# yekaizhou/duet

Measured on AMD Instinct MI355X. Metric: SV support-read marks clustered+phased /sec; bit-exact phased_sv.vcf vs ref, higher is better.
Workload: dtype u32/u64 integer + f64 threshold compares; 1 GPU; BASELINE configs[1]: synthetic 1 contig, 1001116 SV marks / 100000 candidates / 159991 tagged reads, resident in HBM; step = ef_classify + ef_finalize_own, two launches (phasing, E/F; ef_seed_sort 0: ; marks_per_gpu=1001116, candidates_per_gpu=100000, reads_per_gpu=159991, parallelism=contig-sharded x1, svlen_thres=50, suppread_thres=2, device_preheat_steps=2600

## Files before the change

duet_amd/csrc/duet_ef.hip:

```cpp

#include <hip/hip_runtime.h>
#include <hip/hip_ext.h>
#include <stdint.h>
#include <stdio.h>
#include <stdlib.h>
#include <string.h>
#include <string>
#include <vector>

#include "duet_ef.h"
#include "duet_internal.h"

#pragma clang fp contract(off)

namespace {

#ifdef DUET_STAMPS
#define STAMP(k, i) do { if (threadIdx.x == 0 && p.stamps) p.stamps[((size_t)(k) * 65536 + blockIdx.x) * 8 + (i)] = wall_clock64(); } while (0)
#else
#define STAMP(k, i) do { } while (0)
#endif

#include "duet_seeds.hip.h"

// ... 1414 lines not shown
        const bool live = c < n_cands;
        const uint8_t code = live ? p.out_pred[c] : 0;
        const uint32_t ps_in = live ? p.out_ps[c] : 0;
        if (tid == 0) {
            const uint32_t last = min(c0 + 255u, n_cands - 1);
            const uint32_t k0 = (DYN && p.cand_contig) ? (uint32_t)p.cand_contig[c0] : p.blk_ctg[tile];
            uint32_t k1 = k0;
            while (last >= p.ctg_off[k1 + 1]) ++k1;
            uint32_t any = 0;
            for (uint32_t k = k0; k <= k1; ++k) any |= (p.n_one[k] == 0);
            const uint32_t n0 = p.n_one[k0];
            s_meta[0] = k0;
            s_meta[1] = (k0 == k1 && n0 > 0 && n0 <= kOneLds) ? n0 : kEmpty;
            s_meta[2] = any;
            s_meta[3] = p.ctg_off[k0] + k0 + 1;
        }
        __syncthreads();
        STAMP(2, 1);
        const uint32_t k0 = s_meta[0], n_lds = s_meta[1], any_empty = s_meta[2];
        const bool lds_mode = n_lds != kEmpty;
        if (lds_mode) {
            const uint32_t *src = p.onebuf + s_meta[3];
            for (uint32_t i = tid; i < n_lds; i += 256u) s_one[i] = src[i];
            __syncthreads();
        }
        STAMP(2, 2);
        if (live) finalize_candidate(p, c, code, ps_in, k0, lds_mode, s_one, n_lds, any_empty);
        if (!DYN) break;
        __syncthreads();
    }
}

constexpr uint32_t kOwnMaxTiles = 2048;
constexpr uint32_t kOwnTab = 2048;
constexpr uint32_t kOwnKeys = 1024;

struct OwnArgs {
    TileRecs recs;
    const uint64_t *seed_ent, *read_tag;
    const uint32_t *cand_pos, *cand_off, *cand_svread, *cand_refread, *mark_read, *c2rec;
    uint32_t *out_ps, *status;
    uint8_t *out_pred;
    uint32_t c_lo, c_hi;
};

template <class F>
__device__ __forceinline__ void own_each_entry(TileRecs recs, const uint64_t *seed_ent, uint32_t c_lo, uint32_t c_hi, uint32_t first,
                                               uint32_t stride, F f)
{
    const uint32_t b_lo = c_lo / kCandPerBlock, b_hi = (c_hi - 1) / kCandPerBlock;
    for (uint32_t b = b_lo + first; b <= b_hi; b += stride) {
        const ulonglong4 rec = recs[b];
        const uint32_t cnt = (uint32_t)rec.x;
        for (uint32_t j = 0; j < cnt; ++j) {
            const uint64_t e = j == 0 ? rec.y : (j == 1 ? rec.z : (j == 2 ? rec.w : seed_ent[(size_t)b * kCandPerBlock + j]));
            const uint32_t c = (uint32_t)(e >> 32);
            if (c >= c_lo && c < c_hi) f((uint32_t)e);
        }
    }
}

__device__ __forceinline__ uint32_t own_nearest_walk(const OwnArgs &a, uint32_t pos)
{
    uint32_t best = 0;
    int64_t bd = -1;
    own_each_entry(a.recs, a.seed_ent, a.c_lo, a.c_hi, 0u, 1u, [&](uint32_t ps) {
// ... 64 lines not shown
                    ++n;
                    const uint32_t hap = tag_hap(u), pc = tag_pc(u);
                    n1 += hap == 1 ? 1u : 0u; s1 += hap == 1 ? pc : 0u;
                    n2 += hap == 2 ? 1u : 0u; s2 += hap == 2 ? pc : 0u;
                });
                done_ps = g;
                if (n > best) {
                    best = n; ps = g;
                    v.hap1 = n1; v.hap2 = n2; v.t1 = s1; v.t2 = s2;
                    v.hap0 = v.allhap - n1 - n2;
                }
            });
        }
        if (v.hap1 == 0 && v.hap2 == 0) ps = own_nearest_walk(a, c_pos);
        a.out_pred[c] = (uint8_t)decide(2, v, me - mb, a.cand_svread[c], a.cand_refread[c]);
        a.out_ps[c] = ps;
        return;
    }
    a.out_pred[c] = (uint8_t)(code & 3u);
    a.out_ps[c] = own_nearest_walk(a, c_pos);
}

__device__ __forceinline__ uint32_t wave_max_u32(uint32_t v)
{
    v = max(v, (uint32_t)__builtin_amdgcn_update_dpp(0, (int)v, 0xB1, 0xF, 0xF, false));
    v = max(v, (uint32_t)__builtin_amdgcn_update_dpp(0, (int)v, 0x4E, 0xF, 0xF, false));
    v = max(v, (uint32_t)__builtin_amdgcn_update_dpp(0, (int)v, 0x124, 0xF, 0xF, false));
    v = max(v, (uint32_t)__builtin_amdgcn_update_dpp(0, (int)v, 0x128, 0xF, 0xF, false));
    v = max(v, (uint32_t)__builtin_amdgcn_update_dpp(0, (int)v, 0x142, 0xA, 0xF, false));
    v = max(v, (uint32_t)__builtin_amdgcn_update_dpp(0, (int)v, 0x143, 0xC, 0xF, false));
    return (uint32_t)__builtin_amdgcn_readlane((int)v, 63);
}

__device__ __forceinline__ void own_sort_set(const uint32_t *s_tab, uint32_t *s_key, uint32_t *s_one, uint32_t *s_part, uint32_t u)
{
    const uint32_t tid = threadIdx.x, lane = tid & 63u, wave = tid >> 6;
    uint32_t mv[kOwnTab / 256u], cnt = 0;
#pragma unroll
    for (uint32_t j = 0; j < kOwnTab / 256u; ++j) {
        mv[j] = s_tab[tid + 256u * j];
        cnt += mv[j] != kEmpty ? 1u : 0u;
    }
    uint32_t x = cnt;
#pragma unroll
    for (int d = 1; d < 64; d <<= 1) {
        const uint32_t y = __shfl_up(x, d, 64);
        if ((int)lane >= d) x += y;
    }
    if (lane == 63) s_part[wave] = x;
    __syncthreads();
    uint32_t at = x - cnt;
#pragma unroll
    for (uint32_t w = 0; w < 4; ++w) at += w < wave ? s_part[w] : 0u;
#pragma unroll
    for (uint32_t j = 0; j < kOwnTab / 256u; ++j)
        if (mv[j] != kEmpty) s_key[at++] = mv[j];
    const uint32_t U = (u + 63u) & ~63u, nblk = U >> 6;
    if (tid < U - u) s_key[u + tid] = kEmpty;
    __syncthreads();
    for (uint32_t b = wave; b < nblk; b += 4u) s_key[b * 64u + lane] = wave_sort64(s_key[b * 64u + lane], lane);
    __syncthreads();
    for (uint32_t i = tid; i < U; i += 256u) {
        const uint32_t me = s_key[i];
        uint32_t rank = 0;
        for (uint32_t b = 0; b < nblk; b += 4u) {
            const uint32_t *b0 = s_key + b * 64u, *b1 = s_key + min(b + 1u, nblk - 1u) * 64u;
            const uint32_t *b2 = s_key + min(b + 2u, nblk - 1u) * 64u, *b3 = s_key + min(b + 3u, nblk - 1u) * 64u;
            uint32_t p0 = 0, p1 = 0, p2 = 0, p3 = 0;
#pragma unroll
            for (uint32_t st = 32; st > 0; st >>= 1) {
                p0 += b0[p0 + st - 1u] < me ? st : 0u;
                p1 += b1[p1 + st - 1u] < me ? st : 0u;
                p2 += b2[p2 + st - 1u] < me ? st : 0u;
                p3 += b3[p3 + st - 1u] < me ? st : 0u;
            }
            p0 += b0[p0] < me ? 1u : 0u;
            p1 += b1[p1] < me ? 1u : 0u;
            p2 += b2[p2] < me ? 1u : 0u;
            p3 += b3[p3] < me ? 1u : 0u;
            rank += p0 + (b + 1u < nblk ? p1 : 0u) + (b + 2u < nblk ? p2 : 0u) + (b + 3u < nblk ? p3 : 0u);
        }
        if (me != kEmpty) s_one[rank] = me;
    }
    __syncthreads();
}

__device__ __forceinline__ void own_vote_from_marks(const uint32_t *mark_read, const uint64_t *read_tag, uint32_t mb, uint32_t me_,
                                                 const uint32_t *s_tab, Vote *vo, uint32_t *pso)
{
    auto each = [&](auto f) {
        for (uint32_t m0 = mb; m0 < me_; m0 += 8) {
            uint32_t r[8];
            uint64_t t[8];
#pragma unroll
            for (int j = 0; j < 8; ++j) r[j] = mark_read[m0 + j < me_ ? m0 + j : mb];
// ... 26 lines not shown
        uint32_t n = 0, n1 = 0, n2 = 0;
        uint64_t s1 = 0, s2 = 0;
        each([&](uint64_t u) {
            if (u == kUntagged || tag_pc(u) > kPcMax || tag_ps(u) != g) return;
            ++n;
            const uint32_t hap = tag_hap(u), pc = tag_pc(u);
            n1 += hap == 1 ? 1u : 0u; s1 += hap == 1 ? pc : 0u;
            n2 += hap == 2 ? 1u : 0u; s2 += hap == 2 ? pc : 0u;
        });
        done_ps = g;
        if (n > best) {
            best = n; ps = g;
            v.hap1 = n1; v.hap2 = n2; v.t1 = s1; v.t2 = s2;
            v.hap0 = v.allhap - n1 - n2;
        }
    });
    *vo = v;
    *pso = ps;
}

__device__ __forceinline__ bool own_probe(uint32_t *s_tab, uint32_t key, uint32_t h)
{
    for (uint32_t probes = 0; probes < kOwnTab; ++probes) {
        const uint32_t old = atomicCAS(&s_tab[h], kEmpty, key);
        if (old == kEmpty) return true;
        if (old == key) return false;
        h = (h + 1u) & (kOwnTab - 1u);
    }
    return false;
}

constexpr uint32_t kOwnWin = 64;

__global__ __launch_bounds__(256) void ef_finalize_own(const Params p)
{
    __shared__ uint32_t s_tab[kOwnTab];
    __shared__ uint32_t s_key[kOwnKeys];
    __shared__ uint32_t s_one[kOwnKeys];
    __shared__ uint32_t s_win[kOwnWin];
    __shared__ uint32_t s_mm[4][2];
    __shared__ uint32_t s_red[4][3];
    __shared__ uint32_t s_part[4];
    __shared__ uint32_t s_nwin;
    __shared__ __align__(8) uint32_t s_c2[kC2Quota * kC2Words];
    const uint32_t tid = threadIdx.x, lane = tid & 63u, wave = tid >> 6;
    STAMP(2, 0);
    if (blockIdx.x == 0 && tid == 0) p.status[1] = 0;
    const uint32_t n_cands = p.C;
    const uint32_t nK = p.n_small;
    auto coff = [&](uint32_t kk) -> uint32_t { return p.ctg_small[kk]; };
    const uint32_t tile = blockIdx.x;
    const uint32_t c0 = tile * 256u, c = c0 + tid;
    const bool live = c < n_cands;
    const uint32_t cl = live ? c : n_cands - 1u;
    const uint32_t last = min(c0 + 255u, n_cands - 1);
    const uint32_t keys_cap = (p.dbg & DUET_DBG_EF_OWN_SMALLTAB) ? 8u : kOwnKeys;
    const uint32_t win_cap = (p.dbg & DUET_DBG_EF_OWN_SMALLTAB) ? 2u : kOwnWin;
    const TileRecs recs{reinterpret_cast<const ulonglong4 *>(p.blk_rec)};
    constexpr uint32_t kPre = 2;
    static_assert(kPre == 2, "the overflow loop selects between rec[0] and rec[1]");
    ulonglong4 rec[kPre], ext[kPre];
    auto load_recs = [&](uint32_t b_lo, uint32_t b_hi) {
#pragma unroll
        for (uint32_t i = 0; i < kPre; ++i) {
            const uint32_t b = min(b_lo + tid + 256u * i, b_hi);
            rec[i] = recs[b];
            ext[i] = recs.second(b);
        }
    };
    const uint32_t code_ld = p.out_pred[cl], ps_ld = p.out_ps[cl], pos_ld = p.cand_pos[cl];
    const uint32_t o0_ld = p.cand_off[cl], o1_ld = p.cand_off[cl + 1u];
    const uint32_t sv_ld = p.cand_svread[cl], rf_ld = p.cand_refread[cl];
    constexpr uint32_t kPairs = kC2Quota * kC2Words / 2;
    const uint2 *c2src = reinterpret_cast<const uint2 *>(p.c2rec + (size_t)tile * kC2Quota * kC2Words);
    const uint2 a0 = c2src[tid], a1 = c2src[tid + 256u < kPairs ? tid + 256u : tid];
    uint32_t lo = 0, hi = nK;
    while (hi - lo > 1) {
        const uint32_t mid = (lo + hi) >> 1;
        if (coff(mid) <= c0) lo = mid; else hi = mid;
    }
    uint32_t k_first = lo;
    while (k_first < nK && coff(k_first) == coff(k_first + 1)) ++k_first;
    {
        const uint32_t kf = k_first < nK ? k_first : 0u;
        load_recs(coff(kf) / kCandPerBlock, (coff(kf + 1) - 1) / kCandPerBlock);
    }
    asm volatile("" ::"v"(code_ld), "v"(ps_ld), "v"(pos_ld), "v"(o0_ld), "v"(o1_ld), "v"(sv_ld), "v"(rf_ld), "v"(a0.x), "v"(a0.y),
                 "v"(a1.x), "v"(a1.y));
    {
        uint2 *dst = reinterpret_cast<uint2 *>(s_c2);
        dst[tid] = a0;
        if (tid + 256u < kPairs) dst[tid + 256u] = a1;
    }
    const uint32_t code = live ? code_ld : 0u, ps_in = live ? ps_ld : 0u, c_pos = live ? pos_ld : 0u;
    const uint32_t c_o0 = live ? o0_ld : 0u, c_o1 = live ? o1_ld : 0u;
    const uint32_t c_svread = live ? sv_ld : 0u, c_refread = live ? rf_ld : 0u;
    for (uint32_t k = lo; k < nK && coff(k) <= last; ++k) {
        const uint32_t c_lo = coff(k), c_hi = coff(k + 1);
        if (c_lo == c_hi) continue;
        const uint32_t b_lo = c_lo / kCandPerBlock, b_hi = (c_hi - 1) / kCandPerBlock;
        if (k != k_first) load_recs(b_lo, b_hi);
#pragma unroll
        for (uint32_t i = 0; i < kOwnTab / 256u; ++i) s_tab[tid + 256u * i] = kEmpty;
        if (tid == 0) s_nwin = 0;
        const bool mine = live && c >= c_lo && c < c_hi;
        const bool asks = mine && code >= 4u && !(code & kDivZero);
        {
            const uint32_t mn = wave_max_u32(asks ? ~c_pos : 0u), mx = wave_max_u32(asks ? c_pos + 1u : 0u);
            if (lane == 0) { s_mm[wave][0] = mn; s_mm[wave][1] = mx; }
        }
        lds_barrier();
        STAMP(2, 1);
        asm volatile("" ::"v"(rec[0].x), "v"(rec[1].x), "v"(rec[0].y), "v"(rec[1].y), "v"(rec[0].z), "v"(rec[1].z), "v"(rec[0].w),
                     "v"(rec[1].w), "v"(ext[0].x), "v"(ext[1].x), "v"(ext[0].y), "v"(ext[1].y), "v"(ext[0].z), "v"(ext[1].z),
                     "v"(ext[0].w), "v"(ext[1].w));
        uint32_t pmin, pmax;
        {
            const uint32_t a0 = max(max(s_mm[0][0], s_mm[1][0]), max(s_mm[2][0], s_mm[3][0]));
            const uint32_t a1 = max(max(s_mm[0][1], s_mm[1][1]), max(s_mm[2][1], s_mm[3][1]));
            pmin = a1 ? ~a0 : 0u;
            pmax = a1 ? a1 - 1u : 0u;
        }
        uint32_t fresh = 0, leftp = 0, rinv = 0;
        static_assert(kOwnTab == 1u << 11, "the hash takes 11 bits");
        auto slot_of = [](uint32_t key) -> uint32_t { return (key * 2654435761u) >> (32u - 11u); };
        auto count_new = [&](bool nw, uint32_t key) {
            fresh += nw ? 1u : 0u;
            leftp = max(leftp, (nw && key <= pmin) ? key + 1u : 0u);
            rinv = max(rinv, (nw && key >= pmax) ? ~key : 0u);
            if (nw && key > pmin && key < pmax) {
                const uint32_t at = atomicAdd(&s_nwin, 1u);
                if (at < kOwnWin) s_win[at] = key;
            }
        };
        auto insert = [&](uint64_t e) {
            const uint32_t cc = (uint32_t)(e >> 32), key = (uint32_t)e;
            if (cc >= c_lo && cc < c_hi) count_new(own_probe(s_tab, key, slot_of(key)), key);
        };
        uint32_t coll = 0;
        auto group = [&](const uint64_t (&e)[4], uint32_t first, uint32_t n_in, uint32_t cnt, uint32_t bit0) {
            uint32_t key[4], old[4];
            bool ok[4];
#pragma unroll
            for (uint32_t j = 0; j < 4; ++j) {
                const uint32_t cc = (uint32_t)(e[j] >> 32);
                key[j] = (uint32_t)e[j];
                ok[j] = j < n_in && first + j < cnt && cc >= c_lo && cc < c_hi;
                old[j] = kEmpty;
            }
#pragma unroll
            for (uint32_t j = 0; j < 4; ++j)
                if (ok[j]) old[j] = atomicCAS(&s_tab[slot_of(key[j])], kEmpty, key[j]);
#pragma unroll
            for (uint32_t j = 0; j < 4; ++j) {
                coll |= (ok[j] && old[j] != kEmpty && old[j] != key[j]) ? 1u << (bit0 + j) : 0u;
                count_new(ok[j] && old[j] == kEmpty, key[j]);
            }
        };
#pragma unroll
        for (uint32_t i = 0; i < kPre; ++i) {
            const uint32_t cnt = b_lo + tid + 256u * i <= b_hi ? (uint32_t)rec[i].x : 0u;
            if (__any(cnt > 0u)) {
                const uint64_t e[4] = {rec[i].y, rec[i].z, rec[i].w, 0ull};
                group(e, 0u, 3u, cnt, 7u * i);
            }
            if (__any(cnt > 3u)) {
                const uint64_t e[4] = {ext[i].x, ext[i].y, ext[i].z, ext[i].w};
                group(e, 3u, 4u, cnt, 7u * i + 3u);
            }
        }
        while (coll) {
            const uint32_t j = (uint32_t)__ffs(coll) - 1u;
            coll &= coll - 1u;
            uint32_t key = 0;
#pragma unroll
            for (uint32_t i = 0; i < kPre; ++i) {
                key = j == 7u * i + 0u ? (uint32_t)rec[i].y : key;
                key = j == 7u * i + 1u ? (uint32_t)rec[i].z : key;
                key = j == 7u * i + 2u ? (uint32_t)rec[i].w : key;
                key = j == 7u * i + 3u ? (uint32_t)ext[i].x : key;
                key = j == 7u * i + 4u ? (uint32_t)ext[i].y : key;
                key = j == 7u * i + 5u ? (uint32_t)ext[i].z : key;
                key = j == 7u * i + 6u ? (uint32_t)ext[i].w : key;
            }
            count_new(own_probe(s_tab, key, (slot_of(key) + 1u) & (kOwnTab - 1u)), key);
        }
        auto overflow = [&](uint32_t b, uint32_t cnt, uint32_t from) {
            constexpr uint32_t kLong = 24;
            if (cnt > from && cnt <= kLong) {
                const uint64_t *ov = p.seed_ent + (size_t)b * kCandPerBlock;
#pragma unroll 1
                for (uint32_t j = from; j < cnt; j += 4) {
                    uint64_t e[4];
#pragma unroll
                    for (uint32_t t = 0; t < 4; ++t) e[t] = ov[min(j + t, cnt - 1u)];
#pragma unroll
                    for (uint32_t t = 0; t < 4; ++t)
                        if (j + t < cnt) insert(e[t]);
                }
            }
            unsigned long long todo = __ballot(cnt > kLong);
            while (todo) {
                const uint32_t h = (uint32_t)__ffsll((long long)todo) - 1u;
                todo &= todo - 1ull;
                const uint32_t b_h = (uint32_t)__builtin_amdgcn_readlane((int)b, h), cnt_h = (uint32_t)__builtin_amdgcn_readlane((int)cnt, h);
                const uint64_t *ov = p.seed_ent + (size_t)b_h * kCandPerBlock;
                for (uint32_t j = from + lane; j < cnt_h; j += 64u) insert(ov[j]);
            }
        };
#pragma unroll 1
        for (uint32_t i = 0, b0 = b_lo; b0 <= b_hi; ++i, b0 += 256u) {
            const uint32_t b = b0 + tid;
            uint32_t cnt, from = 7u;
            if (i < kPre) {
                cnt = b <= b_hi ? (uint32_t)(i == 0 ? rec[0].x : rec[1].x) : 0u;
            } else {
                ulonglong4 r = {0, 0, 0, 0};
                if (b <= b_hi) r = recs[b];
                cnt = (uint32_t)r.x;
                if (cnt > 0) insert(r.y);
                if (cnt > 1) insert(r.z);
                if (cnt > 2) insert(r.w);
                from = 3u;
            }
            overflow(b, cnt, from);
        }
        {
            const uint32_t l = wave_max_u32(leftp), r = wave_max_u32(rinv), o = wave_sum(fresh);
            if (lane == 0) { s_red[wave][0] = l; s_red[wave][1] = r; s_red[wave][2] = o; }
        }
        lds_barrier();
        STAMP(2, 2);
        const uint32_t u = s_red[0][2] + s_red[1][2] + s_red[2][2] + s_red[3][2];
        const uint32_t Lp = max(max(s_red[0][0], s_red[1][0]), max(s_red[2][0], s_red[3][0]));
        const uint32_t Ri = max(max(s_red[0][1], s_red[1][1]), max(s_red[2][1], s_red[3][1]));
        const uint32_t n_win = s_nwin;
        const bool over = u > keys_cap;
        const bool sorted = !over && n_win > win_cap;
        if (sorted) own_sort_set(s_tab, s_key, s_one, s_part, u);
        STAMP(2, 5);
        auto nearest = [&](uint32_t pos) -> uint32_t {
            if (sorted) return nearest_seed(s_one, u, pos);
            uint32_t best = 0;
            int64_t bd = -1;
            auto look = [&](uint32_t v) {
                const int64_t d = llabs((int64_t)pos - (int64_t)v);
                if (bd < 0 || d < bd || (d == bd && v > best)) { bd = d; best = v; }
            };
            if (Lp) look(Lp - 1u);
            if (Ri) look(~Ri);
            for (uint32_t i = 0; i < n_win; ++i) look(s_win[i]);
            return best;
        };
        auto member = [&](uint32_t key) -> bool {
            uint32_t h = (key * 2654435761u) >> (32u - 11u);
            for (;;) {
                const uint32_t v = s_tab[h];
                if (v == key) return true;
                if (v == kEmpty) return false;
                h = (h + 1u) & (kOwnTab - 1u);
            }
        };
        if (mine) {
            if (u == 0) {
                if (code != 0) p.out_pred[c] = 0;
                if (ps_in != 0) p.out_ps[c] = 0;
            } else if (code >= 4u) {
                if (code & kDivZero) {
                    atomicOr(&p.status[0], 1u);
                    p.out_pred[c] = 0;
                    p.out_ps[c] = 0;
                } else if (over) {
                    const OwnArgs a = {recs, p.seed_ent, p.read_tag, p.cand_pos, p.cand_off, p.cand_svread, p.cand_refread, p.mark_read, p.c2rec,
                                       p.out_ps, p.status, p.out_pred, c_lo, c_hi};
                    finalize_candidate_walk(a, c, code, ps_in);
                } else if (code & kClass2Slow) {
                    Vote v;
                    uint32_t ps;
                    own_vote_from_marks(p.mark_read, p.read_tag, c_o0, c_o1, s_tab, &v, &ps);
                    if (v.hap1 == 0 && v.hap2 == 0) ps = nearest(c_pos);
                    p.out_pred[c] = (uint8_t)decide(2, v, c_o1 - c_o0, c_svread, c_refread);
                    p.out_ps[c] = ps;
                } else if (code & kClass2) {
                    uint32_t w[kC2Words];
                    const uint32_t own0 = tile * kC2Quota;
                    if (ps_in >= own0 && ps_in < own0 + kC2Quota) {
#pragma unroll
                        for (int i = 0; i < kC2Words; ++i) w[i] = s_c2[(ps_in - own0) * kC2Words + i];
                    } else {
                        const uint32_t *rec2 = p.c2rec + (size_t)ps_in * kC2Words;
#pragma unroll
                        for (int i = 0; i < kC2Words; ++i) w[i] = rec2[i];
                    }
                    Vote v = {0, 0, 0, 0, 0, 0};
                    uint32_t ps = 0, best = 0;
                    v.allhap = w[0];
                    const uint32_t ng = w[1];
#pragma unroll
                    for (int g = 0; g < kC2Groups; ++g) {
                        if ((uint32_t)g < ng && w[2 + 6 * g + 1] > best && member(w[2 + 6 * g])) {
                            best = w[2 + 6 * g + 1];
                            ps = w[2 + 6 * g];
                            v.hap1 = w[2 + 6 * g + 2]; v.hap2 = w[2 + 6 * g + 3];
                            v.t1 = w[2 + 6 * g + 4]; v.t2 = w[2 + 6 * g + 5];
                            v.hap0 = v.allhap - v.hap1 - v.hap2;
                        }
                    }
                    if (v.hap1 == 0 && v.hap2 == 0) ps = nearest(c_pos);
                    p.out_pred[c] = (uint8_t)decide(2, v, c_o1 - c_o0, c_svread, c_refread);
                    p.out_ps[c] = ps;
                } else {
                    p.out_pred[c] = (uint8_t)(code & 3u);
                    p.out_ps[c] = nearest(c_pos);
                }
            }
        }
        STAMP(2, 6);
        __syncthreads();
    }
}

__global__ void plan_mark_starts(const uint32_t *ctg_off, uint32_t K, uint8_t *ctg_start)
{
    const uint32_t k = blockIdx.x * blockDim.x + threadIdx.x;
    if (k < K && ctg_off[k] < ctg_off[k + 1]) ctg_start[ctg_off[k]] = 1;
}

__global__ void plan_device(const uint32_t *ctg_off, uint32_t K, uint32_t B, uint32_t *ctg_off_copy, uint32_t *n_one_and_status,
                            uint32_t *blk_ctg)
{
    const uint32_t b = blockIdx.x * blockDim.x + threadIdx.x;
    if (b <= K) ctg_off_copy[b] = ctg_off[b];
    if (b < K + 8) n_one_and_status[b] = 0;
    if (b >= B) return;
    const uint32_t c = b * kCandPerBlock;
    uint32_t lo = 0, hi = K;
    while (hi - lo > 1) {
        const uint32_t mid = (lo + hi) >> 1;
        if (ctg_off[mid] <= c) lo = mid; else hi = mid;
    }
    blk_ctg[b] = lo;
}

__global__ void plan_device_contigs(const uint16_t *cand_contig, const uint32_t *n_cands, uint32_t K, uint32_t B,
                                    uint32_t *ctg_off_copy, uint32_t *n_one_and_status, uint32_t *blk_ctg)
{
    const uint32_t t = blockIdx.x * blockDim.x + threadIdx.x;
    const uint32_t N = *n_cands;
    if (t <= K) {
        uint32_t lo = 0, hi = N;
        while (lo < hi) {
            const uint32_t mid = lo + ((hi - lo) >> 1);
            if (cand_contig[mid] < t) lo = mid + 1; else hi = mid;
// ... 36 lines not shown
    grow = grow || stage_bytes > ctx->plan_stage_cap;
    int rc;
    if (grow) {
        HIP_TRY(ctx, hipDeviceSynchronize());
        for (int i = 0; i < 6; ++i)
            if ((rc = reserve(ctx, *bufs[i], want[i]))) return rc;
        if (stage_bytes > ctx->plan_stage_cap) {
            if (ctx->plan_stage) HIP_TRY(ctx, hipHostFree(ctx->plan_stage));
            ctx->plan_stage = nullptr;
            ctx->plan_stage_cap = 0;
            HIP_TRY(ctx, hipHostMalloc((void **)&ctx->plan_stage, stage_bytes + stage_bytes / 4 + 4096, hipHostMallocDefault));
            ctx->plan_stage_cap = stage_bytes + stage_bytes / 4 + 4096;
        }
    } else {
        HIP_TRY(ctx, hipEventSynchronize(ctx->plan_ev));
    }
    uint32_t *w = (uint32_t *)ctx->ws_small.ptr;
    ctx->d_ctg_off = w;            w += K + 1;
    ctx->d_n_one = w;              w += K;
    ctx->d_status = w;             w += 8;
    ctx->d_blk_ctg = w;            w += B;
    w += ((uintptr_t)w & 63) ? (64 - ((uintptr_t)w & 63)) / 4 : 0;
    ctx->d_blk_cnt = w;
    uint32_t *h_off = ctx->plan_stage, *h_blk = ctx->plan_stage + (K + 1);
    memcpy(h_off, pr->cand_ctg_off, sizeof(uint32_t) * (K + 1));
    {
        uint32_t k = 0;
        for (uint32_t b = 0; b < B; ++b) {
            const uint32_t c = b * kCandPerBlock;
            while (c >= pr->cand_ctg_off[k + 1]) ++k;
            h_blk[b] = k;
        }
    }
    HIP_TRY(ctx, hipMemcpyAsync(ctx->d_ctg_off, h_off, sizeof(uint32_t) * (K + 1), hipMemcpyHostToDevice, stream));
    if (B) HIP_TRY(ctx, hipMemcpyAsync(ctx->d_blk_ctg, h_blk, sizeof(uint32_t) * B, hipMemcpyHostToDevice, stream));
    HIP_TRY(ctx, hipEventRecord(ctx->plan_ev, stream));
    HIP_TRY(ctx, hipMemsetAsync(ctx->d_n_one, 0, sizeof(uint32_t) * ((size_t)K + 8), stream));
    if (C) HIP_TRY(ctx, hipMemsetAsync(ctx->ws_start.ptr, 0, C, stream));
    hipLaunchKernelGGL(plan_mark_starts, dim3((K + 255) / 256), dim3(256), 0, stream, ctx->d_ctg_off, K,
                       (uint8_t *)ctx->ws_start.ptr);
    HIP_TRY(ctx, hipGetLastError());
    ctx->ef_seeds_stale = false;
    ctx->plan_off.assign(pr->cand_ctg_off, pr->cand_ctg_off + K + 1);
    ctx->plan_C = C;
    ctx->plan_stream = stream;
    return DUET_OK;
}

int validate(duet_ctx *ctx, const duet_ef_problem *pr, const void *out_pred, const void *out_ps)
{
    if (!ctx) return fail(nullptr, DUET_ERR_INVALID, "null context");
    if (!pr) return fail(ctx, DUET_ERR_INVALID, "null problem");
    if (!pr->cand_ctg_off) return fail(ctx, DUET_ERR_INVALID, "cand_ctg_off is null");
    if (pr->n_contigs == 0 && pr->n_cands != 0) return fail(ctx, DUET_ERR_INVALID, "candidates without contigs");
    if (pr->cand_ctg_off[0] != 0 || pr->cand_ctg_off[pr->n_contigs] != pr->n_cands)
        return fail(ctx, DUET_ERR_INVALID, "cand_ctg_off must start at 0 and end at n_cands");
    for (uint32_t k = 0; k < pr->n_contigs; ++k)
        if (pr->cand_ctg_off[k] > pr->cand_ctg_off[k + 1])
            return fail(ctx, DUET_ERR_INVALID, "cand_ctg_off must be non-decreasing");
    if (pr->n_cands) {
        if (!pr->cand_pos || !pr->cand_svlen || !pr->cand_svread || !pr->cand_refread || !pr->cand_gt_ok ||
            !pr->cand_off || !pr->mark_read || !out_pred || !out_ps)
            return fail(ctx, DUET_ERR_INVALID, "null array");
        if (pr->n_reads && !pr->read_tag) return fail(ctx, DUET_ERR_INVALID, "read_tag is null");
    }
    return DUET_OK;
}

}

extern "C" {

int duet_abi_version(void) { return DUET_ABI_VERSION; }

const char *duet_last_error(const duet_ctx *ctx) { return ctx ? ctx->err.c_str() : duet_g_last_error.c_str(); }

duet_ctx *duet_ctx_create(int device_id)
// ... 135 lines not shown
    p.c2_cap = (uint32_t)c2_slots((p.C + kCandPerBlock - 1) / kCandPerBlock, p.C);
    p.out_pred = out_pred; p.out_ps = out_ps;
    p.dbg = ctx->dbg;
    p.heavy_t = (ctx->dbg & DUET_DBG_EF_HEAVY_ALL) ? 0u : ((ctx->dbg & DUET_DBG_EF_HEAVY_OFF) ? 0xFFFFFFFFu : ctx->ef_heavy_t);
    p.stamps = ctx->d_stamps;

    hipEvent_t ev[6] = {nullptr, nullptr, nullptr, nullptr, nullptr, nullptr};
    int prof = ctx->profiling;
    if (prof == 3) prof = (ctx->prof_tick++ % 8u == 0) ? 1 : 0;
    if (prof) {
        ctx->ev_mode = prof;
        while (ctx->ev_pool.size() < ctx->ev_used + 6) {
            hipEvent_t e;
            HIP_TRY(ctx, hipEventCreate(&e));
            ctx->ev_pool.push_back(e);
        }
        for (int i = 0; i < (prof == 2 ? 6 : 2); ++i) ev[i] = ctx->ev_pool[ctx->ev_used + i];
        ctx->ev_used += 6;
    }
    const uint32_t blocks = (pr->n_cands + kCandPerBlock - 1) / kCandPerBlock;
    const uint32_t three = DUET_DBG_EF_OWN_OFF | DUET_DBG_EF_FIN_TPB2 | DUET_DBG_EF_FIN_TPB4 | DUET_DBG_EF_NO_SEED_HASH;
    const bool own = p.n_small && !(ctx->dbg & three) && (blocks <= kOwnMaxTiles || (ctx->dbg & DUET_DBG_EF_OWN_ALL));
    const bool split = own && blocks <= kSplitMaxTiles && !(ctx->dbg & DUET_DBG_EF_SPLIT_OFF);
    if (prof) ctx->ev_kmask.push_back(own ? 0x5 : 0x7);
    if (split && ((uintptr_t)pr->mark_read & 15) == 0)
        hipExtLaunchKernelGGL(ef_classify_split<true>, dim3(blocks), dim3(kSplitThreads), 0, stream, ev[0], ev[1], 0, p);
    else if (split)
        hipExtLaunchKernelGGL(ef_classify_split<false>, dim3(blocks), dim3(kSplitThreads), 0, stream, ev[0], ev[1], 0, p);
    else if (((uintptr_t)pr->mark_read & 15) == 0)
        hipExtLaunchKernelGGL(ef_classify<true>, dim3(blocks), dim3(kCandPerBlock), 0, stream, ev[0], ev[1], 0, p);
    else
        hipExtLaunchKernelGGL(ef_classify<false>, dim3(blocks), dim3(kCandPerBlock), 0, stream, ev[0], ev[1], 0, p);
    if (own) {
        hipExtLaunchKernelGGL(ef_finalize_own, dim3(blocks), dim3(256), 0, stream, ev[4], ev[5], 0, p);
        ctx->ef_last_params.assign((const unsigned char *)&p, (const unsigned char *)&p + sizeof(p));
        ctx->ef_last_stream = stream;
        ctx->ef_seeds_stale = true;
    } else {
        ctx->ef_seeds_stale = false;
        hipExtLaunchKernelGGL(ef_seed_sort, dim3(pr->n_contigs), dim3(kSortThreads), 0, stream, ev[2], ev[3], 0, p);
        const uint32_t C = pr->n_cands;
        int tpb = (!p.n_small || C < 1000000u) ? 1 : (C < 8000000u ? 2 : 4);
        if (p.n_small && (ctx->dbg & DUET_DBG_EF_FIN_TPB2)) tpb = 2;
        if (p.n_small && (ctx->dbg & DUET_DBG_EF_FIN_TPB4)) tpb = 4;
        if (tpb == 4) hipExtLaunchKernelGGL((ef_finalize<false, 4>), dim3((C + 1023) / 1024), dim3(256), 0, stream, ev[4], ev[5], 0, p);
        else if (tpb == 2) hipExtLaunchKernelGGL((ef_finalize<false, 2>), dim3((C + 511) / 512), dim3(256), 0, stream, ev[4], ev[5], 0, p);
        else hipExtLaunchKernelGGL((ef_finalize<false, 1>), dim3((C + 255) / 256), dim3(256), 0, stream, ev[4], ev[5], 0, p);
    }
    HIP_TRY(ctx, hipGetLastError());
    ctx->pending_check = true;
    return DUET_OK;
}

}

int duet_ef_plan_on_device_prepare(duet_ctx *ctx, uint32_t K, uint32_t c_max, hipStream_t stream, uint32_t **ctg_off_out,
                                   uint32_t **zero_out)
{
    const uint32_t C = c_max;
    const uint32_t B = (C + kCandPerBlock - 1) / kCandPerBlock;
    const size_t small_words = (size_t)(K + 1) + K + 8 + (size_t)B + 16 + (size_t)B * 16;
    const size_t want[6] = {small_words * 4, C, (size_t)B * kCandPerBlock * 8, ((size_t)C + K + 1) * 4, ((size_t)C + K + 1) * 4,
                            c2_slots(B, C) * kC2Words * 4};
    DevBuf *bufs[6] = {&ctx->ws_small, &ctx->ws_start, &ctx->ws_ent, &ctx->ws_one, &ctx->ws_tmp, &ctx->ws_c2};
    bool grow = ctx->plan_stream != stream;
    for (int i = 0; i < 6; ++i) grow = grow || want[i] > bufs[i]->cap;
    int rc;
    if (grow) {
        HIP_TRY(ctx, hipDeviceSynchronize());
        for (int i = 0; i < 6; ++i)
            if ((rc = reserve(ctx, *bufs[i], want[i]))) return rc;
    }
    uint32_t *w = (uint32_t *)ctx->ws_small.ptr;
    ctx->d_ctg_off = w;            w += K + 1;
    ctx->d_n_one = w;              w += K;
    ctx->d_status = w;             w += 8;
    ctx->d_blk_ctg = w;            w += B;
    w += ((uintptr_t)w & 63) ? (64 - ((uintptr_t)w & 63)) / 4 : 0;
    ctx->d_blk_cnt = w;
    ctx->plan_off.clear();
    ctx->plan_C = 0;
    ctx->plan_stream = stream;
    if (ctg_off_out) *ctg_off_out = ctx->d_ctg_off;
    if (zero_out) *zero_out = ctx->d_n_one;
    return DUET_OK;
}

int duet_ef_run_planned_on_device(duet_ctx *ctx, const duet_ef_problem *pr, uint32_t c_max, const uint32_t *d_n_cands,
                                  const uint32_t *d_ctg_off, const uint16_t *d_cand_contig, uint8_t *out_pred, uint32_t *out_ps,
                                  hipStream_t stream, bool planned)
{
    const uint32_t K = pr->n_contigs, C = c_max;
    if (K == 0 || C == 0) return DUET_OK;
    const uint32_t B = (C + kCandPerBlock - 1) / kCandPerBlock;
    int rc;
    if ((rc = duet_ef_plan_on_device_prepare(ctx, K, c_max, stream, nullptr, nullptr))) return rc;
    if (!planned) {
        const uint32_t nthr = B > K + 8 ? B : K + 8;
        if (d_cand_contig)
            hipLaunchKernelGGL(plan_device_contigs, dim3((nthr + 255) / 256), dim3(256), 0, stream, d_cand_contig, d_n_cands, K, B,
                               ctx->d_ctg_off, ctx->d_n_one, ctx->d_blk_ctg);
        else
            hipLaunchKernelGGL(plan_device, dim3((nthr + 255) / 256), dim3(256), 0, stream, d_ctg_off, K, B, ctx->d_ctg_off,
                               ctx->d_n_one, ctx->d_blk_ctg);
    }

    Params p;
    memset(&p, 0, sizeof(p));
    p.K = K; p.C = C; p.M = pr->n_marks;
    p.dyn_c = d_n_cands;
    p.cand_contig = d_cand_contig;
    p.read_tag = pr->n_reads ? pr->read_tag : (const uint64_t *)ctx->d_n_one;
    p.n_reads = pr->n_reads; p.untagged = ctx->d_untagged;
    p.cand_pos = pr->cand_pos; p.cand_svlen = pr->cand_svlen; p.cand_svread = pr->cand_svread;
// ... 177 lines not shown
```

duet_amd/csrc/duet_internal.h:

```cpp
#ifndef DUET_INTERNAL_H
#define DUET_INTERNAL_H

#include <hip/hip_runtime.h>
#include <stdint.h>
#include <string.h>
#include <algorithm>
#include <string>
#include <vector>

#include "duet_ef.h"

struct DevBuf {
    void *ptr = nullptr;
    size_t cap = 0;
};

struct DuetOwnedBufs {
    DevBuf b[16];
    DuetOwnedBufs() = default;
    DuetOwnedBufs(const DuetOwnedBufs &) = delete;
    DuetOwnedBufs &operator=(const DuetOwnedBufs &) = delete;
    ~DuetOwnedBufs()
    {
        for (DevBuf &x : b)
            if (x.ptr) (void)hipFree(x.ptr);
    }
};

struct duet_ctx {
    int device = 0;
    std::string err;
    int profiling = 0;
    int ev_mode = 0;
    uint32_t prof_tick = 0;
    uint32_t dbg = 0;
    uint32_t ef_heavy_t = 32;
    unsigned long long *d_stamps = nullptr;
    hipStream_t own_stream = nullptr;
    uint64_t *d_untagged = nullptr;
    uint32_t *rx_dtot = nullptr;
    std::vector<uint32_t> plan_off;
    uint32_t plan_C = 0;
    hipStream_t plan_stream = (hipStream_t)-1;
    uint32_t *plan_stage = nullptr;
    size_t plan_stage_cap = 0;
    hipEvent_t plan_ev = nullptr;
    DevBuf ws_small;
    DevBuf ws_start, ws_ent, ws_one, ws_tmp, ws_c2;
    uint32_t *d_ctg_off = nullptr, *d_n_one = nullptr, *d_status = nullptr, *d_blk_ctg = nullptr,
             *d_blk_cnt = nullptr;
    DevBuf h_in[9], h_out[2];
    DevBuf cl_ws[16], cl_in[4], cl_out[6];
    DevBuf rows_ws[8];
    DevBuf rows_in[5];
    DevBuf eval_ws;
    DevBuf sv_ws[5];
    DevBuf sv_in[3], sv_out[2];
    std::vector<uint32_t> sv_depth_off;
    hipStream_t sv_depth_off_stream = nullptr;
    hipEvent_t sv_depth_off_ev = nullptr;
    void *sv_depth_off_at = nullptr;
    hipStream_t cl_side[3] = {nullptr, nullptr, nullptr};
    hipEvent_t cl_fork = nullptr, cl_join[3] = {nullptr, nullptr, nullptr};
    uint32_t *cl_flags = nullptr;
    int cl_gates = 0;
    uint32_t cl_epoch = 0;
    std::vector<hipEvent_t> ev_pool;
    std::vector<uint8_t> ev_kmask;
    size_t ev_used = 0;
    std::vector<unsigned char> ef_last_params;
    hipStream_t ef_last_stream = nullptr;
    bool ef_seeds_stale = false;
    bool pending_check = false;
    DuetOwnedBufs tune_ws;
    DuetOwnedBufs tune_truth_in, tune_truth_out;
// ... 161 lines not shown
```

include/duet_ef.h:

```cpp
#ifndef DUET_EF_H
#define DUET_EF_H

#include <stdint.h>

#ifdef __cplusplus
extern "C" {
#endif

#define DUET_ABI_VERSION 1

#define DUET_API __attribute__((visibility("default")))

typedef enum duet_status {
    DUET_OK = 0,
    DUET_ERR_INVALID = -1,
    DUET_ERR_NO_DEVICE = -2,
    DUET_ERR_HIP = -3,
    DUET_ERR_OOM = -4,
    DUET_ERR_TIMEOUT = -6,
    DUET_ERR_DIV_ZERO = -5
} duet_status;

#define DUET_TAG(hap, pc, ps) (((uint64_t)(hap) << 62) | ((uint64_t)(pc) << 32) | (uint64_t)(uint32_t)(ps))
#define DUET_MARK_ABSENT 0xFFFFFFFFu
// ... 17 lines not shown
    uint32_t suppread_thres;
} duet_ef_problem;

enum { DUET_K_CLASSIFY = 0, DUET_K_SEEDS = 1, DUET_K_FINALIZE = 2, DUET_N_KERNELS = 3 };

typedef struct duet_ef_stats {
    uint64_t algorithmic_bytes;
    uint32_t n_seed_ps;
    uint32_t n_profiled_runs;
    float kernel_ms[DUET_N_KERNELS];
    float total_ms;
} duet_ef_stats;

typedef struct duet_ctx duet_ctx;

DUET_API int duet_abi_version(void);

DUET_API duet_ctx *duet_ctx_create(int device_id);
DUET_API void duet_ctx_destroy(duet_ctx *ctx);
DUET_API const char *duet_last_error(const duet_ctx *ctx);

DUET_API int duet_ctx_set_profiling(duet_ctx *ctx, int mode);

DUET_API int duet_ef_run_device(duet_ctx *ctx, const duet_ef_problem *prob, uint8_t *out_pred, uint32_t *out_ps,
                       void *stream);

DUET_API int duet_ef_check(duet_ctx *ctx, void *stream);

DUET_API int duet_ef_run_host(duet_ctx *ctx, const duet_ef_problem *prob, uint8_t *out_pred, uint32_t *out_ps,
                     duet_ef_stats *stats);

DUET_API int duet_ef_profile_collect(duet_ctx *ctx, duet_ef_stats *stats);

#define DUET_DBG_EF_NO_SEED_HASH 0x40u
#define DUET_DBG_EF_FIN_TPB2 0x20u
#define DUET_DBG_EF_FIN_TPB4 0x80u
#define DUET_DBG_EF_HEAVY_ALL 0x80000u
#define DUET_DBG_EF_HEAVY_OFF 0x100000u
#define DUET_DBG_EF_SPLIT_OFF 0x200000u
#define DUET_DBG_EF_FP_DECIDE 0x400000u
#define DUET_DBG_EF_OWN_OFF 0x800000u
#define DUET_DBG_EF_OWN_ALL 0x1000000u
#define DUET_DBG_EF_OWN_SMALLTAB 0x2000000u
#define DUET_DBG_CLUSTER_EVENT_FORKS 0x4000000u
#define DUET_DBG_CLUSTER_WIDE_OFF 0x8000000u
#define DUET_DBG_CLUSTER_EXACT 0x100u
#define DUET_DBG_CLUSTER_LARGE 0x200u
#define DUET_DBG_CLUSTER_PAIRS 0x400u
#define DUET_DBG_CLUSTER_NOBOX 0x800u
#define DUET_DBG_CLUSTER_KEYSORT 0x10000u
#define DUET_DBG_CLUSTER_RECSORT 0x40000u
#define DUET_DBG_CLUSTER_NOSYM 0x20000u
#define DUET_DBG_CLUSTER_LSD 0x8000u
#define DUET_DBG_CLUSTER_SMALLCAP 0x4000u
#define DUET_DBG_CLUSTER_TIERS 0x2000u
#define DUET_DBG_CLUSTER_KC2 0x1000u
DUET_API int duet_ctx_set_debug(duet_ctx *ctx, uint32_t flags);

DUET_API int duet_ef_get_seed_ps(duet_ctx *ctx, uint32_t contig, uint32_t *out, uint32_t cap);

typedef struct duet_cluster_problem {
    uint32_t n_marks;
    uint32_t part_gap;
    uint32_t part_max;
    uint32_t n_contigs_hint;
    uint32_t n_types_hint;
// ... 389 lines not shown
```

Baseline: 63.21 billion marks/s.

## Add 512-thread two-tile variant of ef_finalize_own for wide single-contig spans

Templates the owner-finalize kernel on a tile multiplier so one 512-thread block handles two candidate tiles. The per-contig hash table of seed records is then built once per pair of tiles instead of once per tile. A host-side plan computes the maximum contig span in blocks and selects the wide kernel when the span is large and the grid is small. The trade is fewer blocks in flight and a larger block footprint in exchange for less redundant per-block table construction.

```diff
diff --git a/duet_amd/csrc/duet_ef.hip b/duet_amd/csrc/duet_ef.hip
--- a/duet_amd/csrc/duet_ef.hip
+++ b/duet_amd/csrc/duet_ef.hip
@@ -1470,6 +1470,7 @@
 }
 
 constexpr uint32_t kOwnMaxTiles = 2048;
+constexpr uint32_t kOwnWideMaxTiles = 512;
 constexpr uint32_t kOwnTab = 2048;
 constexpr uint32_t kOwnKeys = 1024;
 
@@ -1600,13 +1601,15 @@
     return (uint32_t)__builtin_amdgcn_readlane((int)v, 63);
 }
 
+template <uint32_t NT>
 __device__ __forceinline__ void own_sort_set(const uint32_t *s_tab, uint32_t *s_key, uint32_t *s_one, uint32_t *s_part, uint32_t u)
 {
+    constexpr uint32_t NW = NT / 64u;
     const uint32_t tid = threadIdx.x, lane = tid & 63u, wave = tid >> 6;
-    uint32_t mv[kOwnTab / 256u], cnt = 0;
-#pragma unroll
-    for (uint32_t j = 0; j < kOwnTab / 256u; ++j) {
-        mv[j] = s_tab[tid + 256u * j];
+    uint32_t mv[kOwnTab / NT], cnt = 0;
+#pragma unroll
+    for (uint32_t j = 0; j < kOwnTab / NT; ++j) {
+        mv[j] = s_tab[tid + NT * j];
         cnt += mv[j] != kEmpty ? 1u : 0u;
     }
     uint32_t x = cnt;
@@ -1619,16 +1622,16 @@
     __syncthreads();
     uint32_t at = x - cnt;
 #pragma unroll
-    for (uint32_t w = 0; w < 4; ++w) at += w < wave ? s_part[w] : 0u;
-#pragma unroll
-    for (uint32_t j = 0; j < kOwnTab / 256u; ++j)
+    for (uint32_t w = 0; w < NW; ++w) at += w < wave ? s_part[w] : 0u;
+#pragma unroll
+    for (uint32_t j = 0; j < kOwnTab / NT; ++j)
         if (mv[j] != kEmpty) s_key[at++] = mv[j];
     const uint32_t U = (u + 63u) & ~63u, nblk = U >> 6;
     if (tid < U - u) s_key[u + tid] = kEmpty;
     __syncthreads();
-    for (uint32_t b = wave; b < nblk; b += 4u) s_key[b * 64u + lane] = wave_sort64(s_key[b * 64u + lane], lane);
+    for (uint32_t b = wave; b < nblk; b += NW) s_key[b * 64u + lane] = wave_sort64(s_key[b * 64u + lane], lane);
     __syncthreads();
-    for (uint32_t i = tid; i < U; i += 256u) {
+    for (uint32_t i = tid; i < U; i += NT) {
         const uint32_t me = s_key[i];
         uint32_t rank = 0;
         for (uint32_t b = 0; b < nblk; b += 4u) {
@@ -1721,28 +1724,31 @@
 
 constexpr uint32_t kOwnWin = 64;
 
-__global__ __launch_bounds__(256) void ef_finalize_own(const Params p)
-{
+template <uint32_t T>
+__device__ __forceinline__ void finalize_own_tiles(const Params &p)
+{
+    constexpr uint32_t NT = 256u * T, NW = 4u * T;
+    static_assert(kOwnTab % NT == 0 && NT <= 1024u, "the clear and own_sort_set deal the table out evenly");
     __shared__ uint32_t s_tab[kOwnTab];
     __shared__ uint32_t s_key[kOwnKeys];
     __shared__ uint32_t s_one[kOwnKeys];
     __shared__ uint32_t s_win[kOwnWin];
-    __shared__ uint32_t s_mm[4][2];
-    __shared__ uint32_t s_red[4][3];
-    __shared__ uint32_t s_part[4];
+    __shared__ uint32_t s_mm[NW][2];
+    __shared__ uint32_t s_red[NW][3];
+    __shared__ uint32_t s_part[NW];
     __shared__ uint32_t s_nwin;
-    __shared__ __align__(8) uint32_t s_c2[kC2Quota * kC2Words];
+    __shared__ __align__(8) uint32_t s_c2[T * kC2Quota * kC2Words];
     const uint32_t tid = threadIdx.x, lane = tid & 63u, wave = tid >> 6;
     STAMP(2, 0);
     if (blockIdx.x == 0 && tid == 0) p.status[1] = 0;
     const uint32_t n_cands = p.C;
     const uint32_t nK = p.n_small;
     auto coff = [&](uint32_t kk) -> uint32_t { return p.ctg_small[kk]; };
-    const uint32_t tile = blockIdx.x;
-    const uint32_t c0 = tile * 256u, c = c0 + tid;
+    const uint32_t tile = blockIdx.x * T;
+    const uint32_t c0 = blockIdx.x * NT, c = c0 + tid;
     const bool live = c < n_cands;
     const uint32_t cl = live ? c : n_cands - 1u;
-    const uint32_t last = min(c0 + 255u, n_cands - 1);
+    const uint32_t last = min(c0 + (NT - 1u), n_cands - 1);
     const uint32_t keys_cap = (p.dbg & DUET_DBG_EF_OWN_SMALLTAB) ? 8u : kOwnKeys;
     const uint32_t win_cap = (p.dbg & DUET_DBG_EF_OWN_SMALLTAB) ? 2u : kOwnWin;
     const TileRecs recs{reinterpret_cast<const ulonglong4 *>(p.blk_rec)};
@@ -1752,7 +1758,7 @@
     auto load_recs = [&](uint32_t b_lo, uint32_t b_hi) {
 #pragma unroll
         for (uint32_t i = 0; i < kPre; ++i) {
-            const uint32_t b = min(b_lo + tid + 256u * i, b_hi);
+            const uint32_t b = min(b_lo + tid + NT * i, b_hi);
             rec[i] = recs[b];
             ext[i] = recs.second(b);
         }
@@ -1760,9 +1766,10 @@
     const uint32_t code_ld = p.out_pred[cl], ps_ld = p.out_ps[cl], pos_ld = p.cand_pos[cl];
     const uint32_t o0_ld = p.cand_off[cl], o1_ld = p.cand_off[cl + 1u];
     const uint32_t sv_ld = p.cand_svread[cl], rf_ld = p.cand_refread[cl];
-    constexpr uint32_t kPairs = kC2Quota * kC2Words / 2;
+    constexpr uint32_t kPairs = T * kC2Quota * kC2Words / 2;
+    static_assert(kPairs <= 2u * NT, "two pieces per thread");
     const uint2 *c2src = reinterpret_cast<const uint2 *>(p.c2rec + (size_t)tile * kC2Quota * kC2Words);
-    const uint2 a0 = c2src[tid], a1 = c2src[tid + 256u < kPairs ? tid + 256u : tid];
+    const uint2 a0 = c2src[tid], a1 = c2src[tid + NT < kPairs ? tid + NT : tid];
     uint32_t lo = 0, hi = nK;
     while (hi - lo > 1) {
         const uint32_t mid = (lo + hi) >> 1;
@@ -1779,7 +1786,7 @@
     {
         uint2 *dst = reinterpret_cast<uint2 *>(s_c2);
         dst[tid] = a0;
-        if (tid + 256u < kPairs) dst[tid + 256u] = a1;
+        if (tid + NT < kPairs) dst[tid + NT] = a1;
     }
     const uint32_t code = live ? code_ld : 0u, ps_in = live ? ps_ld : 0u, c_pos = live ? pos_ld : 0u;
     const uint32_t c_o0 = live ? o0_ld : 0u, c_o1 = live ? o1_ld : 0u;
@@ -1790,7 +1797,7 @@
         const uint32_t b_lo = c_lo / kCandPerBlock, b_hi = (c_hi - 1) / kCandPerBlock;
         if (k != k_first) load_recs(b_lo, b_hi);
 #pragma unroll
-        for (uint32_t i = 0; i < kOwnTab / 256u; ++i) s_tab[tid + 256u * i] = kEmpty;
+        for (uint32_t i = 0; i < kOwnTab / NT; ++i) s_tab[tid + NT * i] = kEmpty;
         if (tid == 0) s_nwin = 0;
         const bool mine = live && c >= c_lo && c < c_hi;
         const bool asks = mine && code >= 4u && !(code & kDivZero);
@@ -1803,10 +1810,16 @@
         asm volatile("" ::"v"(rec[0].x), "v"(rec[1].x), "v"(rec[0].y), "v"(rec[1].y), "v"(rec[0].z), "v"(rec[1].z), "v"(rec[0].w),
                      "v"(rec[1].w), "v"(ext[0].x), "v"(ext[1].x), "v"(ext[0].y), "v"(ext[1].y), "v"(ext[0].z), "v"(ext[1].z),
                      "v"(ext[0].w), "v"(ext[1].w));
+        STAMP(2, 3);
         uint32_t pmin, pmax;
         {
-            const uint32_t a0 = max(max(s_mm[0][0], s_mm[1][0]), max(s_mm[2][0], s_mm[3][0]));
-            const uint32_t a1 = max(max(s_mm[0][1], s_mm[1][1]), max(s_mm[2][1], s_mm[3][1]));
+            uint32_t a0 = max(max(s_mm[0][0], s_mm[1][0]), max(s_mm[2][0], s_mm[3][0]));
+            uint32_t a1 = max(max(s_mm[0][1], s_mm[1][1]), max(s_mm[2][1], s_mm[3][1]));
+#pragma unroll
+            for (uint32_t w = 4; w < NW; w += 4) {
+                a0 = max(a0, max(max(s_mm[w][0], s_mm[w + 1][0]), max(s_mm[w + 2][0], s_mm[w + 3][0])));
+                a1 = max(a1, max(max(s_mm[w][1], s_mm[w + 1][1]), max(s_mm[w + 2][1], s_mm[w + 3][1])));
+            }
             pmin = a1 ? ~a0 : 0u;
             pmax = a1 ? a1 - 1u : 0u;
         }
@@ -1848,7 +1861,7 @@
         };
 #pragma unroll
         for (uint32_t i = 0; i < kPre; ++i) {
-            const uint32_t cnt = b_lo + tid + 256u * i <= b_hi ? (uint32_t)rec[i].x : 0u;
+            const uint32_t cnt = b_lo + tid + NT * i <= b_hi ? (uint32_t)rec[i].x : 0u;
             if (__any(cnt > 0u)) {
                 const uint64_t e[4] = {rec[i].y, rec[i].z, rec[i].w, 0ull};
                 group(e, 0u, 3u, cnt, 7u * i);
@@ -1898,7 +1911,7 @@
             }
         };
 #pragma unroll 1
-        for (uint32_t i = 0, b0 = b_lo; b0 <= b_hi; ++i, b0 += 256u) {
+        for (uint32_t i = 0, b0 = b_lo; b0 <= b_hi; ++i, b0 += NT) {
             const uint32_t b = b0 + tid;
             uint32_t cnt, from = 7u;
             if (i < kPre) {
@@ -1920,13 +1933,19 @@
         }
         lds_barrier();
         STAMP(2, 2);
-        const uint32_t u = s_red[0][2] + s_red[1][2] + s_red[2][2] + s_red[3][2];
-        const uint32_t Lp = max(max(s_red[0][0], s_red[1][0]), max(s_red[2][0], s_red[3][0]));
-        const uint32_t Ri = max(max(s_red[0][1], s_red[1][1]), max(s_red[2][1], s_red[3][1]));
+        uint32_t u = s_red[0][2] + s_red[1][2] + s_red[2][2] + s_red[3][2];
+        uint32_t Lp = max(max(s_red[0][0], s_red[1][0]), max(s_red[2][0], s_red[3][0]));
+        uint32_t Ri = max(max(s_red[0][1], s_red[1][1]), max(s_red[2][1], s_red[3][1]));
+#pragma unroll
+        for (uint32_t w = 4; w < NW; w += 4) {
+            u += s_red[w][2] + s_red[w + 1][2] + s_red[w + 2][2] + s_red[w + 3][2];
+            Lp = max(Lp, max(max(s_red[w][0], s_red[w + 1][0]), max(s_red[w + 2][0], s_red[w + 3][0])));
+            Ri = max(Ri, max(max(s_red[w][1], s_red[w + 1][1]), max(s_red[w + 2][1], s_red[w + 3][1])));
+        }
         const uint32_t n_win = s_nwin;
         const bool over = u > keys_cap;
         const bool sorted = !over && n_win > win_cap;
-        if (sorted) own_sort_set(s_tab, s_key, s_one, s_part, u);
+        if (sorted) own_sort_set<NT>(s_tab, s_key, s_one, s_part, u);
         STAMP(2, 5);
         auto nearest = [&](uint32_t pos) -> uint32_t {
             if (sorted) return nearest_seed(s_one, u, pos);
@@ -1973,7 +1992,7 @@
                 } else if (code & kClass2) {
                     uint32_t w[kC2Words];
                     const uint32_t own0 = tile * kC2Quota;
-                    if (ps_in >= own0 && ps_in < own0 + kC2Quota) {
+                    if (ps_in >= own0 && ps_in < own0 + T * kC2Quota) {
 #pragma unroll
                         for (int i = 0; i < kC2Words; ++i) w[i] = s_c2[(ps_in - own0) * kC2Words + i];
                     } else {
@@ -2008,6 +2027,10 @@
         __syncthreads();
     }
 }
+
+__global__ __launch_bounds__(256) void ef_finalize_own(const Params p) { finalize_own_tiles<1>(p); }
+
+__global__ __launch_bounds__(512) void ef_finalize_own_wide(const Params p) { finalize_own_tiles<2>(p); }
 
 __global__ void plan_mark_starts(const uint32_t *ctg_off, uint32_t K, uint8_t *ctg_start)
 {
@@ -2110,6 +2133,11 @@
             h_blk[b] = k;
         }
     }
+    uint32_t max_span = 0;
+    for (uint32_t k = 0; k < K; ++k) {
+        const uint32_t c_lo = pr->cand_ctg_off[k], c_hi = pr->cand_ctg_off[k + 1];
+        if (c_lo < c_hi) max_span = std::max(max_span, (c_hi - 1) / kCandPerBlock - c_lo / kCandPerBlock + 1);
+    }
     HIP_TRY(ctx, hipMemcpyAsync(ctx->d_ctg_off, h_off, sizeof(uint32_t) * (K + 1), hipMemcpyHostToDevice, stream));
     if (B) HIP_TRY(ctx, hipMemcpyAsync(ctx->d_blk_ctg, h_blk, sizeof(uint32_t) * B, hipMemcpyHostToDevice, stream));
     HIP_TRY(ctx, hipEventRecord(ctx->plan_ev, stream));
@@ -2121,6 +2149,7 @@
     ctx->ef_seeds_stale = false;
     ctx->plan_off.assign(pr->cand_ctg_off, pr->cand_ctg_off + K + 1);
     ctx->plan_C = C;
+    ctx->plan_max_span = max_span;
     ctx->plan_stream = stream;
     return DUET_OK;
 }
@@ -2322,7 +2351,10 @@
     else
         hipExtLaunchKernelGGL(ef_classify<false>, dim3(blocks), dim3(kCandPerBlock), 0, stream, ev[0], ev[1], 0, p);
     if (own) {
-        hipExtLaunchKernelGGL(ef_finalize_own, dim3(blocks), dim3(256), 0, stream, ev[4], ev[5], 0, p);
+        const bool wide = !(ctx->dbg & DUET_DBG_EF_OWN_NARROW) &&
+                          ((ctx->plan_max_span > 256u && blocks <= kOwnWideMaxTiles) || (ctx->dbg & DUET_DBG_EF_OWN_WIDE));
+        if (wide) hipExtLaunchKernelGGL(ef_finalize_own_wide, dim3((blocks + 1) / 2), dim3(512), 0, stream, ev[4], ev[5], 0, p);
+        else hipExtLaunchKernelGGL(ef_finalize_own, dim3(blocks), dim3(256), 0, stream, ev[4], ev[5], 0, p);
         ctx->ef_last_params.assign((const unsigned char *)&p, (const unsigned char *)&p + sizeof(p));
         ctx->ef_last_stream = stream;
         ctx->ef_seeds_stale = true;
@@ -2370,6 +2402,7 @@
     ctx->d_blk_cnt = w;
     ctx->plan_off.clear();
     ctx->plan_C = 0;
+    ctx->plan_max_span = 0;
     ctx->plan_stream = stream;
     if (ctg_off_out) *ctg_off_out = ctx->d_ctg_off;
     if (zero_out) *zero_out = ctx->d_n_one;
diff --git a/duet_amd/csrc/duet_internal.h b/duet_amd/csrc/duet_internal.h
--- a/duet_amd/csrc/duet_internal.h
+++ b/duet_amd/csrc/duet_internal.h
@@ -41,6 +41,7 @@
     uint32_t *rx_dtot = nullptr;
     std::vector<uint32_t> plan_off;
     uint32_t plan_C = 0;
+    uint32_t plan_max_span = 0;
     hipStream_t plan_stream = (hipStream_t)-1;
     uint32_t *plan_stage = nullptr;
     size_t plan_stage_cap = 0;
diff --git a/include/duet_ef.h b/include/duet_ef.h
--- a/include/duet_ef.h
+++ b/include/duet_ef.h
@@ -73,6 +73,8 @@
 
 DUET_API int duet_ef_profile_collect(duet_ctx *ctx, duet_ef_stats *stats);
 
+#define DUET_DBG_EF_OWN_WIDE 0x1u
+#define DUET_DBG_EF_OWN_NARROW 0x2u
 #define DUET_DBG_EF_NO_SEED_HASH 0x40u
 #define DUET_DBG_EF_FIN_TPB2 0x20u
 #define DUET_DBG_EF_FIN_TPB4 0x80u
```

Measured after the change: 65.44 billion marks/s (median of 6 runs). +3.5%, better.
